# ArchieGertsman/spark-sched-sim

Hardware: AMD Instinct MI355X
Metric: env-steps/sec at 4096 batched envs (TPC-H, 10 exec) (higher is better)
Workload: dtype int64+f64

## Files before the change

spark_sched_sim_amd/csrc/sss_sim_observe.h:

```cpp
#undef SSS_SRC_ID
#define SSS_SRC_ID 10
SSS_DEV int find_schedulable_all() {
  PROF3(21);
  int lane = wave_lane();
  int A = g_sc.m_n_active;
  int src_job = g_sc.m_src_job;
  uint32_t total = 0;
  for (int a0 = 0; a0 < A; a0 += 64) {
    int a = a0 + lane;
    uint32_t cnt = 0;
    if (a < A) {
      int j = lds_active()[a];
      SssJob* job = jobp(j);
      uint64_t m = 0;
      if (j == src_job || (int)job->supply < g_c.E) m = ready_mask_of_job(*job, false);
      job->sched_mask = m;
      cnt = (uint32_t)popc64(m);
    }
    total += wave_sum_u32(cnt);
  }
  return (int)total;
}

SSS_DEV void write_observation(const SssLayout& L, const SssBuffers& B, int env, double reward) {
  PROF3(22);
  int lane = wave_lane();
  uint64_t t_obs0 = wave_clock();
  const SssHdr& h = g_hot.h;
  float* __restrict__ nodes = B.nodes + (size_t)env * L.n_cap * 3;
  int32_t* __restrict__ el = B.edge_links + (size_t)env * L.ed_cap * 2;
  int32_t* __restrict__ dag_ptr = B.dag_ptr + (size_t)env * (L.J_cap + 1);
  int32_t* __restrict__ sup = B.exec_supplies + (size_t)env * L.J_cap;
  int A = h.n_active;
  uint32_t srck = h.curr_source;
  int src_job = (srck == POOL_NONE || srck == POOL_COMMON) ? -1 : key_job(srck);
  int src_idx = A;
  uint64_t lt = bit64(lane) - 1;
  uint16_t* nbase = lds_keys();
  uint32_t run = 0;
  for (int a0 = 0; a0 < A; a0 += 64) {
    int a = a0 + lane;
    uint32_t cnt = 0;
    int j = -1, supply = 0;
    if (a < A) {
      j = lds_active()[a];
      const SssJob* job = jobp(j);
      cnt = (uint32_t)popc64(job->active_mask);
      supply = job->supply;
    }
    uint32_t excl = wave_scan_excl_u32(cnt);
    uint32_t tot = wave_sum_u32(cnt);
    uint64_t is_src = wave_ballot(a < A && j == src_job);
    if (is_src) src_idx = a0 + ctz64(is_src);
    if (a < A) {
      nbase[a] = (uint16_t)(run + excl);
      dag_ptr[a] = (int32_t)(run + excl);
      sup[a] = supply;
    }
    run += tot;
  }
  int base_n = (int)run;
  wave_sync();
  int SPn = g_c.SP;
  for (int i0 = lane; i0 < A * SPn; i0 += 64 * 4) {
    int32_t remaining[4];
    float recent[4];
    uint64_t act[4], sched[4];
    int nst[4];
    SSS_UNROLL4 for (int u = 0; u < 4; u++) {
      const int i = i0 + 64 * u;
      remaining[u] = 0, recent[u] = 0.0f, act[u] = 0, sched[u] = 0, nst[u] = 0;
      if (i < A * SPn) {
        const int a = i / SPn, st = i - a * SPn;
        const JobView v = jobview(lds_active()[a]);
        remaining[u] = v.st[st].remaining;
        recent[u] = v.dur[st];
        act[u] = v.job->active_mask, sched[u] = v.job->sched_mask, nst[u] = (int)v.job->n_stages;
      }
    }
    SSS_UNROLL4 for (int u = 0; u < 4; u++) {
      const int i = i0 + 64 * u;
      if (i < A * SPn) {
        const int a = i / SPn, st = i - a * SPn;
        if (st < nst[u] && (act[u] & bit64(st))) {
          const int row = (int)nbase[a] + popc64(act[u] & (bit64(st) - 1));
          nodes[row * 3 + 0] = (float)remaining[u];
          nodes[row * 3 + 1] = recent[u];
          nodes[row * 3 + 2] = (sched[u] & bit64(st)) ? 1.0f : 0.0f;
        }
      }
    }
  }
  const bool same_graph = h.obs_graph_version == h.graph_version && h.obs_bind_gen == B.gen;
  int ME = g_c.P.max_edges;
  int base_e = same_graph ? h.obs_n_edges : 0;
  for (int i0 = 0; i0 < (same_graph ? 0 : A * ME); i0 += 64 * 4) {
    uint64_t act[4];
    int eoff[4], nb[4];
    bool has[4];
    SSS_UNROLL4 for (int u = 0; u < 4; u++) {
      const int i = i0 + 64 * u + lane;
      has[u] = false, act[u] = 0, eoff[u] = 0, nb[u] = 0;
      if (i < A * ME) {
        const int a = i / ME, e = i - a * ME;
        const SssJob* job = jobp(lds_active()[a]);
        has[u] = e < (int)job->n_edges;
        act[u] = job->active_mask, eoff[u] = job->edge_off + e, nb[u] = (int)nbase[a];
      }
    }
    int uu[4], vv[4];
    SSS_UNROLL4 for (int u = 0; u < 4; u++) {
      uu[u] = 0, vv[u] = 0;
      if (has[u]) uu[u] = g_c.pk.edges[2 * eoff[u]], vv[u] = g_c.pk.edges[2 * eoff[u] + 1];
    }
    SSS_UNROLL4 for (int u = 0; u < 4; u++) {
      if (i0 + 64 * u >= A * ME) break;
      const bool keep = has[u] && (act[u] & bit64(uu[u])) && (act[u] & bit64(vv[u]));
      const uint64_t bal = wave_ballot(keep);
      if (keep) {
        const int pos = base_e + popc64(bal & lt);
        el[2 * pos + 0] = nb[u] + popc64(act[u] & (bit64(uu[u]) - 1));
        el[2 * pos + 1] = nb[u] + popc64(act[u] & (bit64(vv[u]) - 1));
      }
      base_e += popc64(bal);
    }
  }
  if (lane == 0) {
    dag_ptr[A] = base_n;
    int32_t* oi = B.obs_i32 + (size_t)env * SSS_OBS_I32;
    double* of = B.obs_f64 + (size_t)env * SSS_OBS_F64;
    int ncommit = 0;
    if (srck != POOL_NONE) {
      int p = pool_index(srck);
      ncommit = (int)g_c.pool_hdr[p].used - (int)g_c.pool_hdr[p].commit_from;
    }
    oi[OBS_N_NODES] = base_n, oi[OBS_N_EDGES] = base_e, oi[OBS_N_JOBS] = A, oi[OBS_N_SCHED] = h.n_sched;
    oi[OBS_NUM_COMMITTABLE] = ncommit, oi[OBS_SOURCE_JOB_IDX] = src_idx;
    oi[OBS_TERMINATED] = h.terminated, oi[OBS_ERR] = h.err;
    of[OBS_REWARD] = reward, of[OBS_WALL_TIME] = h.wall_time;
    g_hot.h.prof[4] += wave_clock() - t_obs0;
    g_hot.h.obs_n_nodes = base_n;
    g_hot.h.obs_graph_version = h.graph_version, g_hot.h.obs_n_edges = base_e, g_hot.h.obs_bind_gen = B.gen;
    g_hot.h.obs_n_sched = h.n_sched;
    g_hot.h.last_reward = reward;
    g_hot.h.model_bytes += (uint64_t)g_sc.events_this_step * 140u + 24u * (uint64_t)base_n + 4u * (uint64_t)(A + 1) +
                            4u * (uint64_t)A + 8u * (uint64_t)base_e + 12u + 26u;
  }
}
```

Baseline: 24.07 million.

## Compact observation writer to active-stage iteration with per-chunk LDS scratch and prefix search

Restructures write_observation so each 64-job chunk stages active masks, edge offsets, job location and packed node/edge prefix sums in LDS scratch. Lanes then iterate over only the real stage slots and real edges, found by binary search over the prefixes, instead of over A*SP and A*max_edges padded slots. Job and stage data are read through address-space-qualified pointers from the LDS cache when the job is cached, and from HBM otherwise. The pool used/commit_from pair is loaded as one word early so its latency is hidden. The cost is reused scratch areas in g_sc, an extra wave_sync per chunk, and more complex indexing.

```diff
diff --git a/spark_sched_sim_amd/csrc/sss_sim_observe.h b/spark_sched_sim_amd/csrc/sss_sim_observe.h
--- a/spark_sched_sim_amd/csrc/sss_sim_observe.h
+++ b/spark_sched_sim_amd/csrc/sss_sim_observe.h
@@ -1,5 +1,6 @@
 #undef SSS_SRC_ID
 #define SSS_SRC_ID 10
+#include <stddef.h>
 SSS_DEV int find_schedulable_all() {
   PROF3(21);
   int lane = wave_lane();
@@ -20,6 +21,41 @@
     total += wave_sum_u32(cnt);
   }
   return (int)total;
+}
+
+#define OBS_ACT_LO ((uint32_t*)g_sc.setA)
+#define OBS_ACT_HI ((uint32_t*)g_sc.setB)
+#define OBS_EOFF (g_sc.fc_dst)
+#define OBS_PREF (g_sc.rl_old)
+#define OBS_LOC (g_sc.rl_seq)
+#define OBS_EPREF ((uint16_t*)g_sc.fc_num)
+#define OBS_LOC_HBM 0x80000000u
+#define OBS_NO_ROW 0xFFFFFFFFu
+#define OBS_PREF_END 0xFFFFu
+static_assert(offsetof(SssPoolHdr, commit_from) == offsetof(SssPoolHdr, used) + 2 && offsetof(SssPoolHdr, used) % 4 == 0, "used and commit_from are read as one word");
+static_assert(SSS_SET_TABLE >= 256 && SSS_MAX_EXEC >= 64, "the observation writer's per-job scratch is 64 entries of 4 bytes per area");
+
+#if defined(__HIP_DEVICE_COMPILE__)
+#define SSS_AS_LDS(T, p) ((const __attribute__((address_space(3))) T*)(p))
+#define SSS_AS_HBM(T, p) ((const __attribute__((address_space(1))) T*)(p))
+#define SSS_USE_HERE(x) asm volatile("" : "+v"(x))
+#else
+#define SSS_AS_LDS(T, p) ((const T*)(p))
+#define SSS_AS_HBM(T, p) ((const T*)(p))
+#define SSS_USE_HERE(x) ((void)(x))
+#endif
+
+SSS_DEV int obs_find_by_slot(int i) {
+  int lo = 0;
+  SSS_UNROLL8 for (int w = 32; w >= 1; w >>= 1)
+    if ((int)(OBS_PREF[lo + w] & 0xFFFFu) <= i) lo += w;
+  return lo;
+}
+SSS_DEV int obs_find_by_edge(int i) {
+  int lo = 0;
+  SSS_UNROLL8 for (int w = 32; w >= 1; w >>= 1)
+    if ((int)OBS_EPREF[lo + w] <= i) lo += w;
+  return lo;
 }
 
 SSS_DEV void write_observation(const SssLayout& L, const SssBuffers& B, int env, double reward) {
@@ -33,107 +69,141 @@
   int32_t* __restrict__ sup = B.exec_supplies + (size_t)env * L.J_cap;
   int A = h.n_active;
   uint32_t srck = h.curr_source;
+  uint32_t src_used_cf = 0;
+  if (A == 0 && lane == 0 && srck != POOL_NONE) src_used_cf = *SSS_AS_HBM(uint32_t, &g_c.pool_hdr[pool_index(srck)].used);
   int src_job = (srck == POOL_NONE || srck == POOL_COMMON) ? -1 : key_job(srck);
   int src_idx = A;
   uint64_t lt = bit64(lane) - 1;
-  uint16_t* nbase = lds_keys();
+  const bool same_graph = h.obs_graph_version == h.graph_version && h.obs_bind_gen == B.gen;
+  int base_e = same_graph ? h.obs_n_edges : 0;
+  const int SPn = g_c.SP;
   uint32_t run = 0;
   for (int a0 = 0; a0 < A; a0 += 64) {
-    int a = a0 + lane;
-    uint32_t cnt = 0;
+    const int a = a0 + lane;
+    uint32_t cnt = 0, nst = 0, ned = 0, loc = 0, eoff = 0;
+    uint64_t act = 0;
     int j = -1, supply = 0;
     if (a < A) {
       j = lds_active()[a];
-      const SssJob* job = jobp(j);
-      cnt = (uint32_t)popc64(job->active_mask);
-      supply = job->supply;
-    }
-    uint32_t excl = wave_scan_excl_u32(cnt);
-    uint32_t tot = wave_sum_u32(cnt);
+      const int s = lds_slot_of()[j];
+      if (a == 0 && srck != POOL_NONE) src_used_cf = *SSS_AS_HBM(uint32_t, &g_c.pool_hdr[pool_index(srck)].used);
+      if (s != SLOT_NONE) {
+        const auto* job = SSS_AS_LDS(SssJob, lds_cjobs()) + s;
+        act = job->active_mask, supply = job->supply, nst = job->n_stages, ned = job->n_edges, eoff = (uint32_t)job->edge_off;
+        loc = (uint32_t)s;
+      } else {
+        const auto* job = SSS_AS_HBM(SssJob, g_c.jobs) + j;
+        act = job->active_mask, supply = job->supply, nst = job->n_stages, ned = job->n_edges, eoff = (uint32_t)job->edge_off;
+        loc = OBS_LOC_HBM | (uint32_t)j;
+      }
+      cnt = (uint32_t)popc64(act);
+    }
+    const uint32_t both = cnt << 16 | nst;
+    const uint32_t excl = wave_scan_excl_u32(both);
+    const uint32_t tot = wave_readlane_u32(excl + both, 63);
+    uint32_t e_excl = 0, tot_e = 0;
+    if (!same_graph) {
+      e_excl = wave_scan_excl_u32(ned);
+      tot_e = wave_readlane_u32(e_excl + ned, 63);
+    }
     uint64_t is_src = wave_ballot(a < A && j == src_job);
     if (is_src) src_idx = a0 + ctz64(is_src);
     if (a < A) {
-      nbase[a] = (uint16_t)(run + excl);
-      dag_ptr[a] = (int32_t)(run + excl);
+      OBS_ACT_LO[lane] = (uint32_t)act, OBS_ACT_HI[lane] = (uint32_t)(act >> 32);
+      OBS_EOFF[lane] = eoff, OBS_LOC[lane] = loc;
+      OBS_PREF[lane] = excl, OBS_EPREF[lane] = (uint16_t)e_excl;
+    } else {
+      OBS_PREF[lane] = OBS_PREF_END, OBS_EPREF[lane] = (uint16_t)OBS_PREF_END;
+    }
+    wave_sync();
+    const int tot_s = (int)(tot & 0xFFFFu);
+    for (int i0 = 0; i0 < tot_s; i0 += 64 * 4) {
+      uint32_t info[4], lc[4];
+      int32_t remaining[4];
+      float recent[4];
+      uint32_t sched[4];
+      SSS_UNROLL4 for (int u = 0; u < 4; u++) {
+        const int i = i0 + 64 * u + lane;
+        info[u] = OBS_NO_ROW, lc[u] = 0;
+        if (i < tot_s) {
+          const int al = obs_find_by_slot(i);
+          const uint32_t pref = OBS_PREF[al];
+          const int st = i - (int)(pref & 0xFFFFu);
+          const uint64_t am = (uint64_t)OBS_ACT_HI[al] << 32 | OBS_ACT_LO[al];
+          if (am & bit64(st)) {
+            info[u] = (run + (pref >> 16) + (uint32_t)popc64(am & (bit64(st) - 1))) | (uint32_t)st << 20;
+            lc[u] = OBS_LOC[al];
+            if (lc[u] & OBS_LOC_HBM) {
+              const int jj = (int)(lc[u] & ~OBS_LOC_HBM);
+              remaining[u] = SSS_AS_HBM(SssStage, g_c.stages)[jj * SPn + st].remaining;
+              recent[u] = SSS_AS_HBM(float, g_c.durations)[jj * SPn + st];
+              sched[u] = SSS_AS_HBM(uint32_t, &g_c.jobs[jj].sched_mask)[st >> 5];
+            }
+          }
+        }
+      }
+      SSS_UNROLL4 for (int u = 0; u < 4; u++) {
+        if (info[u] != OBS_NO_ROW && !(lc[u] & OBS_LOC_HBM)) {
+          const int row = (int)(info[u] & 0xFFFFFu), st = (int)(info[u] >> 20), s = (int)lc[u];
+          nodes[row * 3 + 0] = (float)SSS_AS_LDS(SssStage, lds_cstages())[s * SPn + st].remaining;
+          nodes[row * 3 + 1] = SSS_AS_LDS(float, lds_cdur())[s * SPn + st];
+          nodes[row * 3 + 2] = (SSS_AS_LDS(uint32_t, &lds_cjobs()[s].sched_mask)[st >> 5] >> (st & 31) & 1u) ? 1.0f : 0.0f;
+        }
+      }
+      SSS_UNROLL4 for (int u = 0; u < 4; u++) {
+        SSS_USE_HERE(remaining[u]);
+        SSS_USE_HERE(recent[u]);
+        SSS_USE_HERE(sched[u]);
+      }
+      SSS_UNROLL4 for (int u = 0; u < 4; u++) {
+        if (info[u] != OBS_NO_ROW && (lc[u] & OBS_LOC_HBM)) {
+          const int row = (int)(info[u] & 0xFFFFFu), st = (int)(info[u] >> 20);
+          nodes[row * 3 + 0] = (float)remaining[u];
+          nodes[row * 3 + 1] = recent[u];
+          nodes[row * 3 + 2] = (sched[u] >> (st & 31) & 1u) ? 1.0f : 0.0f;
+        }
+      }
+    }
+    for (int i0 = 0; i0 < (int)tot_e; i0 += 64 * 4) {
+      int al[4], uu[4], vv[4];
+      SSS_UNROLL4 for (int u = 0; u < 4; u++) {
+        const int i = i0 + 64 * u + lane;
+        al[u] = -1, uu[u] = 0, vv[u] = 0;
+        if (i < (int)tot_e) {
+          al[u] = obs_find_by_edge(i);
+          const int eo = (int)OBS_EOFF[al[u]] + (i - (int)OBS_EPREF[al[u]]);
+          uu[u] = g_c.pk.edges[2 * eo], vv[u] = g_c.pk.edges[2 * eo + 1];
+        }
+      }
+      SSS_UNROLL4 for (int u = 0; u < 4; u++) {
+        if (i0 + 64 * u >= (int)tot_e) break;
+        uint64_t am = 0;
+        int nb = 0;
+        if (al[u] >= 0) am = (uint64_t)OBS_ACT_HI[al[u]] << 32 | OBS_ACT_LO[al[u]], nb = (int)(run + (OBS_PREF[al[u]] >> 16));
+        const bool keep = (am & bit64(uu[u])) && (am & bit64(vv[u]));
+        const uint64_t bal = wave_ballot(keep);
+        if (keep) {
+          const int pos = base_e + popc64(bal & lt);
+          el[2 * pos + 0] = nb + popc64(am & (bit64(uu[u]) - 1));
+          el[2 * pos + 1] = nb + popc64(am & (bit64(vv[u]) - 1));
+        }
+        base_e += popc64(bal);
+      }
+    }
+    if (a < A) {
+      dag_ptr[a] = (int32_t)(run + (excl >> 16));
       sup[a] = supply;
     }
-    run += tot;
+    run += tot >> 16;
+    if (a0 + 64 < A) wave_sync();
   }
   int base_n = (int)run;
-  wave_sync();
-  int SPn = g_c.SP;
-  for (int i0 = lane; i0 < A * SPn; i0 += 64 * 4) {
-    int32_t remaining[4];
-    float recent[4];
-    uint64_t act[4], sched[4];
-    int nst[4];
-    SSS_UNROLL4 for (int u = 0; u < 4; u++) {
-      const int i = i0 + 64 * u;
-      remaining[u] = 0, recent[u] = 0.0f, act[u] = 0, sched[u] = 0, nst[u] = 0;
-      if (i < A * SPn) {
-        const int a = i / SPn, st = i - a * SPn;
-        const JobView v = jobview(lds_active()[a]);
-        remaining[u] = v.st[st].remaining;
-        recent[u] = v.dur[st];
-        act[u] = v.job->active_mask, sched[u] = v.job->sched_mask, nst[u] = (int)v.job->n_stages;
-      }
-    }
-    SSS_UNROLL4 for (int u = 0; u < 4; u++) {
-      const int i = i0 + 64 * u;
-      if (i < A * SPn) {
-        const int a = i / SPn, st = i - a * SPn;
-        if (st < nst[u] && (act[u] & bit64(st))) {
-          const int row = (int)nbase[a] + popc64(act[u] & (bit64(st) - 1));
-          nodes[row * 3 + 0] = (float)remaining[u];
-          nodes[row * 3 + 1] = recent[u];
-          nodes[row * 3 + 2] = (sched[u] & bit64(st)) ? 1.0f : 0.0f;
-        }
-      }
-    }
-  }
-  const bool same_graph = h.obs_graph_version == h.graph_version && h.obs_bind_gen == B.gen;
-  int ME = g_c.P.max_edges;
-  int base_e = same_graph ? h.obs_n_edges : 0;
-  for (int i0 = 0; i0 < (same_graph ? 0 : A * ME); i0 += 64 * 4) {
-    uint64_t act[4];
-    int eoff[4], nb[4];
-    bool has[4];
-    SSS_UNROLL4 for (int u = 0; u < 4; u++) {
-      const int i = i0 + 64 * u + lane;
-      has[u] = false, act[u] = 0, eoff[u] = 0, nb[u] = 0;
-      if (i < A * ME) {
-        const int a = i / ME, e = i - a * ME;
-        const SssJob* job = jobp(lds_active()[a]);
-        has[u] = e < (int)job->n_edges;
-        act[u] = job->active_mask, eoff[u] = job->edge_off + e, nb[u] = (int)nbase[a];
-      }
-    }
-    int uu[4], vv[4];
-    SSS_UNROLL4 for (int u = 0; u < 4; u++) {
-      uu[u] = 0, vv[u] = 0;
-      if (has[u]) uu[u] = g_c.pk.edges[2 * eoff[u]], vv[u] = g_c.pk.edges[2 * eoff[u] + 1];
-    }
-    SSS_UNROLL4 for (int u = 0; u < 4; u++) {
-      if (i0 + 64 * u >= A * ME) break;
-      const bool keep = has[u] && (act[u] & bit64(uu[u])) && (act[u] & bit64(vv[u]));
-      const uint64_t bal = wave_ballot(keep);
-      if (keep) {
-        const int pos = base_e + popc64(bal & lt);
-        el[2 * pos + 0] = nb[u] + popc64(act[u] & (bit64(uu[u]) - 1));
-        el[2 * pos + 1] = nb[u] + popc64(act[u] & (bit64(vv[u]) - 1));
-      }
-      base_e += popc64(bal);
-    }
-  }
   if (lane == 0) {
     dag_ptr[A] = base_n;
     int32_t* oi = B.obs_i32 + (size_t)env * SSS_OBS_I32;
     double* of = B.obs_f64 + (size_t)env * SSS_OBS_F64;
-    int ncommit = 0;
-    if (srck != POOL_NONE) {
-      int p = pool_index(srck);
-      ncommit = (int)g_c.pool_hdr[p].used - (int)g_c.pool_hdr[p].commit_from;
-    }
+    SSS_USE_HERE(src_used_cf);
+    const int ncommit = (int)(uint16_t)src_used_cf - (int)(int16_t)(src_used_cf >> 16);
     oi[OBS_N_NODES] = base_n, oi[OBS_N_EDGES] = base_e, oi[OBS_N_JOBS] = A, oi[OBS_N_SCHED] = h.n_sched;
     oi[OBS_NUM_COMMITTABLE] = ncommit, oi[OBS_SOURCE_JOB_IDX] = src_idx;
     oi[OBS_TERMINATED] = h.terminated, oi[OBS_ERR] = h.err;
```

Measured after the change: 24.61 million, median of 6. 2.3% higher.
